# IseanB/SensorFusion-KalmanFilter

Measured on AMD Instinct MI355X. Metric: KF predict+update steps/sec (batched filters), higher is better.
Workload: dtype f64

## Files before the change

include/kf.h:

```cpp
#ifndef KFMI_KF_H
#define KFMI_KF_H

#include <stdint.h>

#ifdef __cplusplus
extern "C" {
#endif

#define KF_OK        0
#define KF_EINVAL   (-1)
#define KF_EHIP     (-2)
#define KF_ENOTSPD  (-3)
#define KF_ENODEV   (-4)
#define KF_ENOMEM   (-5)

#define KF_F32 0
#define KF_F64 1

#define KF_MODEL_CV2 2
#define KF_MODEL_CV3 3

#define KF_MODEL_REF15 15

#define KF_MODEL_REF8 8
// ... 104 lines not shown
#define KF_SCORE_IMU_N        3
#define KF_SCORE_IMU_NIS      4
#define KF_SCORE_IMU_LOGDET_S 5
#define KF_SCORE_POS_N        6
#define KF_SCORE_POS_SSE      7
#define KF_SCORE_ROWS         8
int kf_run_sweep_scores(kf_batch* handle, int T, const uint8_t* etype, const double* dt, const void* payload,
                        const double* thresholds, const double* consts, const double* track, double* scores,
                        void* traj, void* logdet, uint8_t* updated, int32_t* n_updated,
                        int ckpt_every, void* ckpt_x, void* ckpt_P, void* stream);

int kf_smooth_sweep(kf_batch* handle, int T, const uint8_t* etype, const double* dt, const double* consts,
                    const void* filt_x, const void* filt_P, void* sm_x, void* sm_P, void* sm_traj,
                    void* sm_logdet, int32_t* sm_status, void* stream);

int kf_consts_rows(int model, int* rows);

int kf_run_tails(kf_batch* handle, int T, const uint8_t* etype, const double* dt, const void* payload,
                 const int32_t* lo, const int32_t* hi, const double* thresholds,
                 const void* src_x, const void* src_P, int src_rows, int64_t src_batch,
                 const int32_t* src_row, const int32_t* src_col,
                 int32_t* n_updated, void* stream);

int kf_stream_check(kf_batch* handle, double* out, void* stream);

int kf_eval_combos(kf_batch* handle, int n_events, const double* events, const double* init,
                   double prev_time, double target_end, int k, uint64_t combo_offset, void* logdets,
                   void* max_logdet, int32_t* n_records, void* stream);

int kf_search_combos(kf_batch* handle, int n_events, const double* events, const double* init,
// ... 82 lines not shown
```

sensorfusion-kalmanfilter_amd/csrc/kf_capi.cpp:

```cpp
#include <hip/hip_runtime.h>

#include <algorithm>
#include <cmath>
#include <climits>
#include <cstdarg>
#include <cstdlib>
#include <cstdio>
#include <cstring>
#include <mutex>
#include <string>
#include <vector>

#include "../../include/kf.h"
#include "kf_internal.h"

struct kf_batch {
    int model;
    int axes;
    int n, m, c;
    int np;
    int dtype;
    int64_t B;
    int device;
    kf_params params;
// ... 34 lines not shown
    int64_t search_info[4];
    uint64_t* search_host;
    uint64_t* search_host_dev;
    bool search_ctr_zero;
    hipStream_t search_ctr_stream;
    void* win_ws;
    size_t win_ws_bytes;
    bool win_ws_graph;
    uint64_t* win_host;
    uint64_t* win_host_dev;
    size_t win_host_words;
    void* tails_ws;
    size_t tails_ws_bytes;
    bool tails_ws_graph;
    std::vector<kfmi::TailSpec> tails_host;
    void* sch_ws;
    size_t sch_ws_bytes;
    bool sch_ws_graph;
    uint64_t* sch_host;
    uint64_t* sch_host_dev;
    std::vector<double> sch_cand;
};

namespace {

thread_local std::string g_err;

int fail(int code, const char* fmt, ...) __attribute__((format(printf, 2, 3)));
int fail(int code, const char* fmt, ...) {
    char buf[512];
// ... 293 lines not shown
        case KF_OPT_STREAM_CHUNKS: ok = value == 0 || (value >= 2 && value <= (int64_t(1) << 24)); break;
        case KF_OPT_START_THREADS: ok = value == 0 || (value >= 1 && value <= kfmi::kBlock); break;
        case KF_OPT_SEARCH_KERNEL: ok = value >= 0 && value <= 2; break;
        default: return fail(KF_EINVAL, "kf_set_option: unknown option %d", option);
    }
    if (!ok) return fail(KF_EINVAL, "kf_set_option: value %lld out of range for option %d", (long long)value, option);
    h->opt[option] = value;
    return KF_OK;
}

int kf_get_option(const kf_batch* h, int option, int64_t* value) {
    if (int rc = check_handle(h)) return rc;
    if (option < 1 || option >= KF_OPT_COUNT) return fail(KF_EINVAL, "kf_get_option: unknown option %d", option);
    if (!value) return fail(KF_EINVAL, "kf_get_option: null output");
    *value = h->opt[option];
    return KF_OK;
}

const char* kf_last_error(void) { return g_err.c_str(); }

int kf_default_params(int model, kf_params* out) {
    const int d = model_axes(model);
    if (!d) return fail(KF_EINVAL, "unknown model %d", model);
    if (!out) return fail(KF_EINVAL, "null params");
    std::memset(out, 0, sizeof *out);
    if (is_ref(model)) {
        ref_default_consts(model, out);
        return KF_OK;
    }
    out->q_pos = 5.0;
// ... 143 lines not shown
    if (h->P) (void)hipFree(h->P);
    if (h->status) (void)hipFree(h->status);
    if (h->ws) (void)hipFree(h->ws);
    if (h->ws_evt) (void)hipEventDestroy(h->ws_evt);
    if (h->search_ws) (void)hipFree(h->search_ws);
    if (h->search_host) (void)hipHostFree(h->search_host);
    if (h->win_ws) (void)hipFree(h->win_ws);
    if (h->win_host) (void)hipHostFree(h->win_host);
    if (h->flag) (void)hipFree(h->flag);
    if (h->stream_ws) (void)hipFree(h->stream_ws);
    if (h->pend_u) (void)hipFree(h->pend_u);
    if (h->pend_done) (void)hipEventDestroy(h->pend_done);
    if (h->kc) (void)hipFree(h->kc);
    if (h->sched_ws) (void)hipFree(h->sched_ws);
    if (h->tails_ws) (void)hipFree(h->tails_ws);
    if (h->sch_ws) (void)hipFree(h->sch_ws);
    if (h->sch_host) (void)hipHostFree(h->sch_host);
    for (auto& r : h->retired) (void)hipFree(r.first);
    delete h;
    return KF_OK;
}

int kf_release_retired(kf_batch* h, int64_t* bytes_freed) {
    if (int rc = check_handle(h)) return rc;
    int64_t freed = 0;
    for (auto& r : h->retired) {
        (void)hipFree(r.first);
        freed += static_cast<int64_t>(r.second);
    }
    h->retired.clear();
// ... 379 lines not shown
    return run_sweep_impl("kf_run_sweep_params", h, T, etype, dt, payload, thresholds, consts, traj, logdet, updated,
                          n_updated, ckpt_every, ckpt_x, ckpt_P, stream);
}

int kf_run_sweep_scores(kf_batch* h, int T, const uint8_t* etype, const double* dt, const void* payload,
                        const double* thresholds, const double* consts, const double* track, double* scores,
                        void* traj, void* logdet, uint8_t* updated, int32_t* n_updated, int ckpt_every, void* ckpt_x,
                        void* ckpt_P, void* stream) {
    if (int rc = check_handle(h)) return rc;
    if (!consts) return fail(KF_EINVAL, "kf_run_sweep_scores: null consts (a table is mandatory; equal columns for one set)");
    if (!scores) return fail(KF_EINVAL, "kf_run_sweep_scores: null scores");
    return run_sweep_impl("kf_run_sweep_scores", h, T, etype, dt, payload, thresholds, consts, traj, logdet, updated,
                          n_updated, ckpt_every, ckpt_x, ckpt_P, stream, track, scores);
}

int kf_smooth_sweep(kf_batch* h, int T, const uint8_t* etype, const double* dt, const double* consts,
                    const void* filt_x, const void* filt_P, void* sm_x, void* sm_P, void* sm_traj, void* sm_logdet,
                    int32_t* sm_status, void* stream) {
    const char* fn = "kf_smooth_sweep";
    if (int rc = check_handle(h)) return rc;
    if (!is_ref(h)) return fail(KF_EINVAL, "%s: needs a KF_MODEL_REF15 or KF_MODEL_REF8 handle", fn);
    if (h->dtype != KF_F64) return fail(KF_EINVAL, "%s: needs an f64 handle (the f32 smoother is not built)", fn);
    if (T < 0) return fail(KF_EINVAL, "%s: T = %d < 0", fn, T);
    if (T == 0 || h->B == 0) return KF_OK;
    if (!etype || !dt || !filt_x || !filt_P) return fail(KF_EINVAL, "%s: null etype/dt/filt_x/filt_P", fn);
    if (uint64_t(T) * 8u >= (uint64_t(1) << 32))
        return fail(KF_EINVAL, "%s: T = %d events exceed the 4 GiB dt descriptor (8 T)", fn, T);
    if (uint64_t(h->B) * 27u * 8u >= (uint64_t(1) << 31))
        return fail(KF_EINVAL, "%s: B = %lld filters exceed the 2 GiB row span (27 B 8)", fn, (long long)h->B);
    const int model = h->model == KF_MODEL_REF15 ? 15 : 8;
// ... 2 lines not shown
                    kfmi::consts_rows(model));
    kfmi::SmoothArgs a{};
    a.B = h->B;
    a.T = T;
    a.etype = etype;
    a.dt = dt;
    a.filt_x = filt_x;
    a.filt_P = filt_P;
    a.sm_x = sm_x;
    a.sm_P = sm_P;
    a.sm_traj = sm_traj;
    a.sm_logdet = sm_logdet;
    a.sm_status = sm_status;
    a.kc = h->kc;
    a.consts = consts;
    hipError_t e = kfmi::launch_ref_smooth(model, a, static_cast<hipStream_t>(stream));
    return e == hipSuccess ? KF_OK : hip_fail(e, fn);
}

int kf_consts_rows(int model, int* rows) {
    if (!is_ref(model))
        return fail(KF_EINVAL, "kf_consts_rows: model %d has no per-filter constants (KF_MODEL_REF15 or KF_MODEL_REF8)",
                    model);
    if (!rows) return fail(KF_EINVAL, "kf_consts_rows: null rows");
    *rows = kfmi::consts_rows(model == KF_MODEL_REF15 ? 15 : 8);
    return KF_OK;
}

int kf_run_tails(kf_batch* h, int T, const uint8_t* etype, const double* dt, const void* payload, const int32_t* lo,
                 const int32_t* hi, const double* thresholds, const void* src_x, const void* src_P, int src_rows,
                 int64_t src_batch, const int32_t* src_row, const int32_t* src_col, int32_t* n_updated, void* stream) {
    if (int rc = check_handle(h)) return rc;
// ... 1106 lines not shown
```

sensorfusion-kalmanfilter_amd/csrc/kf_internal.h:

```cpp
#pragma once

#include <hip/hip_runtime.h>
#include <stdint.h>

namespace kfmi {

struct CvArgs {
    int64_t B;
    int T;
    int update_every;
    double dt;
    const double* dt_steps;
    const double* dt_filter;
    void* x;
    void* P;
    int32_t* status;
    const void* u;
    const void* x0;
    const void* z;
    const uint8_t* mask;
    void* traj;
    void* logdet;
    double q_pos, q_vel;
    double r[6];
// ... 95 lines not shown
};
static_assert(sizeof(int64_t) == sizeof(double*), "scores shares src_B's slot");
enum : int {
    kScoreGpsN = 0,
    kScoreGpsNis = 1,
    kScoreGpsLogdetS = 2,
    kScoreImuN = 3,
    kScoreImuNis = 4,
    kScoreImuLogdetS = 5,
    kScorePosN = 6,
    kScorePosSse = 7,
    kScoreRows = 8
};
constexpr int consts_rows(int model) { return model == 15 ? 33 : 18; }

struct SmoothArgs {
    int64_t B;
    int T;
    const uint8_t* etype;
    const double* dt;
    const void* filt_x;
    const void* filt_P;
    void* sm_x;
    void* sm_P;
    void* sm_traj;
    void* sm_logdet;
    int32_t* sm_status;
    const RefConsts* kc;
    const double* consts;
};

struct StreamCheck {
    int32_t ok;
    int32_t bad;
    double cov_gap;
    double state_gap;
    int32_t done;
    int32_t pad;
    int32_t skip_chain;
    int32_t skip_gated;
};
struct StreamArgs {
    int64_t C;
    double delta;
// ... 208 lines not shown
    bool rec_time;
};

enum class Op { Run, Predict, Update, Step, Reset };

hipError_t launch_cv(int axes, bool f64, Op op, const CvArgs& a, hipStream_t stream);
hipError_t launch_cv_offblock(int axes, bool f64, const CvArgs& a, int* flag, hipStream_t stream);
hipError_t launch_synth(int axes, bool f64, const SynthArgs& a, hipStream_t stream);
hipError_t launch_copy(void* dst, const void* src, size_t bytes, hipStream_t stream);
constexpr int kEventsLane = 0, kEventsChain = 1, kEventsLds = 2, kEventsGated = 3;
hipError_t launch_ref_events(int model, bool f64, const RefArgs& a, hipStream_t stream, int variant);
hipError_t launch_ref_stream(int model, bool f64, const RefArgs& a, hipStream_t stream, int nv = 1);
hipError_t launch_ref_sweep(int model, bool f64, const SweepArgs& a, hipStream_t stream, bool scored = false);
hipError_t launch_ref_tails(int model, bool f64, const SweepArgs& a, hipStream_t stream);
hipError_t launch_ref_smooth(int model, const SmoothArgs& a, hipStream_t stream);
hipError_t launch_ref_reset(int model, bool f64, const RefArgs& a, hipStream_t stream);
hipError_t launch_ref15_combos(bool f64, const Ref15ComboArgs& a, hipStream_t stream);
hipError_t launch_ref15_search(bool f64, const Ref15SearchArgs& a, bool child_major, hipStream_t stream);
hipError_t launch_ref15_search_pair(bool f64, const Ref15SearchArgs& a, bool child_major, hipStream_t stream);
void set_search_band(Ref15SearchArgs& a, bool f64);
hipError_t launch_ref15_search_head(bool f64, const Ref15SearchArgs& a, hipStream_t stream);
hipError_t launch_ref15_search_end(bool f64, const Ref15SearchArgs& a, hipStream_t stream);
hipError_t launch_ref15_search_windows(bool f64, bool sym, const Ref15WindowArgs* wins, int W, uint64_t max_lanes,
                                       int n_max, int k_max, const uint64_t* binom, const RefConsts* kc,
                                       hipStream_t stream);
hipError_t launch_search_windows_finish(const Ref15WindowArgs* wins, int W, int k_max, uint64_t* host,
                                        hipStream_t stream);
hipError_t launch_search_finish(uint64_t* counters, uint64_t* host, int n, bool zero, hipStream_t stream);
hipError_t launch_ref15_score(bool f64, const Ref15ScoreArgs& a, hipStream_t stream);
hipError_t launch_ref15_scheduled(bool f64, const Ref15SchedArgs& a, hipStream_t stream);
// ... 10 lines not shown
```

sensorfusion-kalmanfilter_amd/csrc/kf_ref.hip:

```cpp
#include <hip/hip_runtime.h>
#include <stdint.h>

#include <cmath>
#include <cstdlib>
#include <cstring>
#include <type_traits>

#include "kf_common.h"
#include "kf_internal.h"

namespace kfmi {
namespace {

template <typename T>
__device__ __forceinline__ __attribute__((address_space(4))) const T* ro(const T* p) {
    return (__attribute__((address_space(4))) const T*)p;
}
typedef __attribute__((address_space(4))) const double ro_double;
typedef __attribute__((address_space(4))) const uint64_t ro_u64;

using namespace dev;

constexpr int kGps = 0, kImu = 1;
constexpr int kRefNewton = 1;
// ... 1256 lines not shown
        row[kScorePosSse] = group_sum(pva ? sc.sse : 0.0);
        const auto rs = span_rsrc(a.scores, 0, uint32_t(a.B) * 8u, kScoreRows);
#pragma unroll
        for (int r = 0; r < kScoreRows; ++r) {
            const bool count = r == kScoreGpsN || r == kScoreImuN || r == kScorePosN;
            stv(rs, c == 0 ? (uint32_t(r) * uint32_t(a.B) + uint32_t(f)) * 8u : kDropOffset,
                bad && !count ? nan : row[r]);
        }
    }
}

#ifndef KF_SMOOTH_DEPTH
#define KF_SMOOTH_DEPTH KF_SWEEP_DEPTH
#endif
constexpr int kSmoothDepth = KF_SMOOTH_DEPTH;

template <typename T>
struct SmoothIn {
    int type;
    double dt;
    T x[3], P[6];
};

template <bool PARAMS>
__device__ __forceinline__ auto smooth_consts(const SmoothArgs& a, int64_t f) {
    if constexpr (PARAMS) return ConstsColumn{a.consts, a.B, f};
    else return a.kc;
}

template <typename T, class M, bool CUSTOM, bool PARAMS = false>
__global__ __launch_bounds__(kSweepBlock) void ref_smooth_kernel(const SmoothArgs a) {
    static_assert(!PARAMS || !CUSTOM, "per-filter constants in place of the handle's");
    const int64_t g = static_cast<int64_t>(blockIdx.x) * kSweepBlock + threadIdx.x;
    const int64_t f = g / kGroup;
    if (f >= a.B) return;
    const ChainLane<T, M, CUSTOM> L(static_cast<int>(g % kGroup), smooth_consts<PARAMS>(a, f));
    const int c = L.c;
    const bool live = L.live;
    const uint32_t off = uint32_t(f) * uint32_t(sizeof(T));
    const uint32_t rb = uint32_t(a.B) * uint32_t(sizeof(T));
    uint32_t vx[3], vp[6];
#pragma unroll
    for (int k = 0; k < 3; ++k) vx[k] = L.xi[k] >= 0 ? uint32_t(L.xi[k]) * rb + off : kDropOffset;
#pragma unroll
    for (int k = 0; k < 6; ++k) vp[k] = L.pr[k] >= 0 ? uint32_t(L.pr[k]) * rb + off : kDropOffset;
    const uint32_t v_tr = (L.xi[0] >= 0 && L.xi[0] < M::NTRAJ) ? uint32_t(L.xi[0]) * rb + off : kDropOffset;
    const uint32_t v_ld = c == 0 ? off : kDropOffset;
    const bool need_x = a.sm_x != nullptr, need_P = a.sm_P != nullptr;
    const bool need_tr = a.sm_traj != nullptr, need_ld = a.sm_logdet != nullptr;

    const int T_ = a.T;
    const uint32_t S = uint32_t(T_);
    const auto r_et = bytes_rsrc(a.etype, S), r_dt = bytes_rsrc(a.dt, S * 8u);
    auto load_row = [&](int t, T (&x)[3], T (&P)[6]) {
        const auto rx = span_rsrc(a.filt_x, int64_t(t) * M::N, rb, M::N);
        const auto rp = span_rsrc(a.filt_P, int64_t(t) * M::NBLK, rb, M::NBLK);
#pragma unroll
        for (int k = 0; k < 3; ++k) x[k] = ldv(rx, vx[k], T(0));
#pragma unroll
        for (int k = 0; k < 6; ++k) P[k] = L.pr[k] >= 0 ? ldv(rp, vp[k], T(0)) : L.unit(k);
    };
    auto is_nan_row = [&](const T (&x)[3], const T (&P)[6]) {
        bool nan = false;
#pragma unroll
        for (int k = 0; k < 3; ++k) nan = nan || x[k] != x[k];
#pragma unroll
        for (int k = 0; k < 6; ++k) nan = nan || P[k] != P[k];
        return nan;
    };
    int32_t st = 0;
    T xs[1][3], Ps[6];
    auto poison = [&]() {
        st = kNotSpd;
#pragma unroll
        for (int k = 0; k < 3; ++k) xs[0][k] = quiet_nan<T>();
#pragma unroll
        for (int k = 0; k < 6; ++k) Ps[k] = quiet_nan<T>();
    };
    auto store_row = [&](int t) {
        if (need_x) {
            const auto rx = span_rsrc(a.sm_x, int64_t(t) * M::N, rb, M::N);
#pragma unroll
            for (int k = 0; k < 3; ++k) stv(rx, vx[k], xs[0][k]);
        }
        if (need_P) {
            const auto rp = span_rsrc(a.sm_P, int64_t(t) * M::NBLK, rb, M::NBLK);
#pragma unroll
            for (int k = 0; k < 6; ++k) stv(rp, vp[k], Ps[k]);
        }
        if (need_tr) stv(span_rsrc(a.sm_traj, int64_t(t) * M::NTRAJ, rb, M::NTRAJ), v_tr, xs[0][0]);
        if (need_ld) {
            const T ld = group_sum(live ? chain_log_det(Ps) : T(0));
            stv(span_rsrc(a.sm_logdet, t, rb, 1), v_ld, ld);
        }
    };

    load_row(T_ - 1, xs[0], Ps);
    __builtin_amdgcn_s_waitcnt(0);
    if (group_any(live && is_nan_row(xs[0], Ps))) poison();
    store_row(T_ - 1);

    const int n = T_ - 1;
    auto load = [&](int s, SmoothIn<T>& in) {
        const int t = T_ - 2 - (s < n ? s : n - 1);
        in.type = int(__builtin_amdgcn_raw_buffer_load_b8(r_et, uint32_t(t + 1), 0, 0));
        in.dt = ldv(r_dt, uint32_t(t + 1) * 8u, 0.0);
        load_row(t, in.x, in.P);
    };
    auto step = [&](int s, const SmoothIn<T>& in) {
        const int t = T_ - 2 - s;
        const int type = wave_uniform(in.type);
        bool bad = is_nan_row(in.x, in.P);
        if (type != 255) {
            const T dt = T(in.dt);
            T xp[1][3] = {{in.x[0], in.x[1], in.x[2]}};
            T Pp[6], FP[3][3];
#pragma unroll
            for (int k = 0; k < 6; ++k) Pp[k] = in.P[k];
            L.template predict<1>(dt, xp, Pp, FP);
            const T d0 = Pp[0];
            const T i0 = T(1) / d0;
            const T l10 = Pp[1] * i0, l20 = Pp[2] * i0;
            const T v0 = l10 * d0;
            const T d1 = fmaT(-l10, v0, Pp[3]);
            const T i1 = T(1) / d1;
            const T l21 = fmaT(-l20, v0, Pp[4]) * i1;
            const T d2 = fmaT(-l21, l21 * d1, fmaT(-l20, l20 * d0, Pp[5]));
            const T i2 = T(1) / d2;
            bad = bad || !(d0 > T(0) && d1 > T(0) && d2 > T(0));
            T C[3][3];
#pragma unroll
            for (int i = 0; i < 3; ++i) {
                const T w0 = FP[0][i];
                const T w1 = fmaT(-l10, w0, FP[1][i]);
                const T w2 = fmaT(-l21, w1, fmaT(-l20, w0, FP[2][i]));
                const T c2 = w2 * i2;
                const T c1 = fmaT(-l21, c2, w1 * i1);
                const T c0 = fmaT(-l20, c2, fmaT(-l10, c1, w0 * i0));
                C[i][0] = c0, C[i][1] = c1, C[i][2] = c2;
            }
            T dx[3], D[6];
#pragma unroll
            for (int k = 0; k < 3; ++k) dx[k] = xs[0][k] - xp[0][k];
#pragma unroll
            for (int k = 0; k < 6; ++k) D[k] = Ps[k] - Pp[k];
#pragma unroll
            for (int i = 0; i < 3; ++i)
                xs[0][i] = fmaT(C[i][2], dx[2], fmaT(C[i][1], dx[1], fmaT(C[i][0], dx[0], in.x[i])));
            T CD[3][3];
#pragma unroll
            for (int i = 0; i < 3; ++i)
#pragma unroll
                for (int j = 0; j < 3; ++j)
                    CD[i][j] = fmaT(C[i][2], D[tri<3>(2, j)], fmaT(C[i][1], D[tri<3>(1, j)], C[i][0] * D[tri<3>(0, j)]));
#pragma unroll
            for (int i = 0; i < 3; ++i)
#pragma unroll
                for (int j = i; j < 3; ++j)
                    Ps[tri<3>(i, j)] =
                        fmaT(CD[i][2], C[j][2], fmaT(CD[i][1], C[j][1], fmaT(CD[i][0], C[j][0], in.P[tri<3>(i, j)])));
            if (!L.pva) {
                xs[0][2] = T(0);
                Ps[2] = Ps[4] = T(0);
                Ps[5] = T(1);
            }
        }
        if (group_any(live && bad) || st != 0) poison();
        store_row(t);
    };
    ring_run<kSmoothDepth, T, SmoothIn<T>>(n, load, step);
    if (a.sm_status) {
        const auto rs = span_rsrc(a.sm_status, 0, uint32_t(a.B) * 4u, 1);
        __builtin_amdgcn_raw_buffer_store_b32(uint32_t(st), rs, c == 0 ? uint32_t(f) * 4u : kDropOffset, 0, 0);
    }
}

template <typename T, class M, bool CUSTOM>
__global__ __launch_bounds__(64) void ref_chain_gated_kernel(const RefArgs a) {
    if (a.skip && *a.skip) return;
    const int lane = int(threadIdx.x);
    const int slot = lane / kGroup;
    const ChainLane<T, M, CUSTOM> L(lane & (kGroup - 1), a.kc);
    const int c = L.c, ia = L.ia, ib = L.ib;
    const bool pva = L.pva, live = L.live;
    const auto& xi = L.xi;
    const auto& pr = L.pr;
// ... 2969 lines not shown
    if (scored && (!a.consts || !a.scores)) return hipErrorInvalidValue;
    const dim3 grid(static_cast<unsigned>((a.B * kGroup + kSweepBlock - 1) / kSweepBlock));
    if (a.consts && scored)
        KF_MODEL_DISPATCH(model, f64,
                          ref_sweep_kernel<T, M, false, false, true, true><<<grid, kSweepBlock, 0, stream>>>(a));
    else if (a.consts)
        KF_MODEL_DISPATCH(model, f64, ref_sweep_kernel<T, M, false, false, true><<<grid, kSweepBlock, 0, stream>>>(a));
    else
        KF_REF_DISPATCH(model, f64, a.kc, ref_sweep_kernel<T, M, CUSTOM><<<grid, kSweepBlock, 0, stream>>>(a));
    return hipGetLastError();
}

hipError_t launch_ref_smooth(int model, const SmoothArgs& a, hipStream_t stream) {
    if (a.B <= 0 || a.T <= 0 || (model != 15 && model != 8) || !a.filt_x || !a.filt_P || !a.etype || !a.dt)
        return hipErrorInvalidValue;
    const dim3 grid(static_cast<unsigned>((a.B * kGroup + kSweepBlock - 1) / kSweepBlock));
    if (a.consts)
        KF_MODEL_DISPATCH(model, true, if constexpr (sizeof(T) == 8)
                                           ref_smooth_kernel<T, M, false, true><<<grid, kSweepBlock, 0, stream>>>(a));
    else
        KF_REF_DISPATCH(model, true, a.kc, if constexpr (sizeof(T) == 8)
                                               ref_smooth_kernel<T, M, CUSTOM><<<grid, kSweepBlock, 0, stream>>>(a));
    return hipGetLastError();
}

template <typename T, class M>
void stream_phase(int phase, const StreamArgs& a, hipStream_t stream) {
    constexpr int NCH = M::NP + M::NA;
    auto grid = [](int64_t n) { return dim3(static_cast<unsigned>((n + kBlock - 1) / kBlock)); };
    switch (phase) {
        case 0: stream_init_kernel<T, M><<<grid(a.C), kBlock, 0, stream>>>(a); break;
        case 1: stream_perturb_kernel<T, M><<<grid(4 * a.C), kBlock, 0, stream>>>(a); break;
        case kStreamPhaseScanTiles: {
            const dim3 g(unsigned((a.C + kScanTile - 1) / kScanTile), NCH);
            stream_scan_tiles_kernel<T, M><<<g, kScanTile, 0, stream>>>(a);
            break;
        }
// ... 303 lines not shown
```

sensorfusion-kalmanfilter_amd/kfmi/_lib.py:

```python
from __future__ import annotations

import ctypes
import glob
import hashlib
import os
import re

HERE = os.path.dirname(os.path.abspath(__file__))
LIB_PATH = os.path.abspath(os.environ.get('KFMI_LIB') or os.path.join(HERE, 'libkfmi.so'))
HEADER = os.path.normpath(os.path.join(HERE, '..', '..', 'include', 'kf.h'))
CSRC = os.path.normpath(os.path.join(HERE, '..', 'csrc'))

KF_OK = 0
KF_EINVAL = -1
KF_EHIP = -2
KF_ENOTSPD = -3
KF_ENODEV = -4
KF_ENOMEM = -5
KF_F32 = 0
KF_F64 = 1
KF_MODEL_CV2 = 2
KF_MODEL_CV3 = 3
KF_MODEL_REF15 = 15
KF_MODEL_REF8 = 8
# ... 82 lines not shown
    'kf_set_state': (_i, [_vp, _vp, _vp, _i, _vp]),
    'kf_get_state': (_i, [_vp, _vp, _vp, _i, _vp]),
    'kf_get_status': (_i, [_vp, _vp, _i, _vp]),
    'kf_predict': (_i, [_vp, _d, _vp, _vp, _vp, _vp]),
    'kf_update': (_i, [_vp, _vp, _vp, _vp, _vp]),
    'kf_run': (_i, [_vp, _i, _d, _vp, _vp, _vp, _vp, _i, _vp, _vp, _vp]),
    'kf_synth': (_i, [_vp, ctypes.c_uint64, _i64, _i, _d, _i, _vp, _vp, _vp, _vp]),
    'kf_run_events': (_i, [_vp, _i, _vp, _vp, _vp, _vp, _vp, _vp, _vp, _i, _d, _vp]),
    'kf_run_events_seq': (_i, [_vp, _i, _vp, _vp, _vp, _vp, _vp, _vp, _vp, _i, _d, _vp]),
    'kf_run_events_gates': (_i, [_vp, _i, _vp, _vp, _vp, _vp, _vp, _vp, _vp, _vp, _vp]),
    'kf_run_stream': (_i, [_vp, _i, _vp, _vp, _vp, _vp, _vp, _vp, _vp, _i, _i, _vp]),
    'kf_run_sweep': (_i, [_vp, _i, _vp, _vp, _vp, _vp, _vp, _vp, _vp, _vp, _i, _vp, _vp, _vp]),
    'kf_run_sweep_params': (_i, [_vp, _i, _vp, _vp, _vp, _vp, _vp, _vp, _vp, _vp, _vp, _i, _vp, _vp, _vp]),
    'kf_run_sweep_scores': (_i, [_vp, _i, _vp, _vp, _vp, _vp, _vp, _vp, _vp, _vp, _vp, _vp, _vp, _i, _vp, _vp, _vp]),
    'kf_smooth_sweep': (_i, [_vp, _i, _vp, _vp, _vp, _vp, _vp, _vp, _vp, _vp, _vp, _vp, _vp]),
    'kf_consts_rows': (_i, [_i, ctypes.POINTER(_i)]),
    'kf_run_tails': (_i, [_vp, _i, _vp, _vp, _vp, _vp, _vp, _vp, _vp, _vp, _i, _i64, _vp, _vp, _vp, _vp]),
    'kf_stream_check': (_i, [_vp, _vp, _vp]),
    'kf_eval_combos': (_i, [_vp, _i, _vp, _vp, _d, _d, _i, ctypes.c_uint64, _vp, _vp, _vp, _vp]),
    'kf_search_combos': (_i, [_vp, _i, _vp, _vp, _d, _d, _d, _i, _i, _i, ctypes.c_uint64,
                              ctypes.POINTER(ctypes.c_uint64), ctypes.POINTER(_i), _vp, _vp, _vp]),
    'kf_search_windows': (_i, [_vp, _i, _i, _vp, _vp, _vp, _vp, _vp, _vp, _i, _vp, _vp, _vp, _vp]),
    'kf_search_schedules': (_i, [_vp, _i, _vp, _vp, _vp, _vp, _d, _i, _vp, ctypes.POINTER(ctypes.c_uint64),
                                 ctypes.POINTER(_d), ctypes.POINTER(ctypes.c_uint64), _vp, _vp]),
    'kf_schedule_plan': (_i, [_vp, _i, _vp, _i, _vp]),
    'kf_search_plan': (_i,[_vp, _i, _vp, _i, ctypes.c_uint64, _i, _vp]),
    'kf_search_info': (_i, [_vp, _vp]),
    'kf_score_candidates': (_i, [_vp, _i, _vp, _i, _vp, _vp, _vp]),
    'kf_score_rows': (_i, [_vp, _i, _vp, _vp, _vp, _vp, _vp]),
    'kf_run_scheduled': (_i, [_vp, _i, _vp, _vp, _vp, _vp, _vp, _d, _vp, _vp, _vp, _vp, _vp]),
# ... 89 lines not shown
```

sensorfusion-kalmanfilter_amd/kfmi/engine.py:

```python
from __future__ import annotations

import collections
import ctypes
import math

import numpy as np
import torch

from . import _lib
from ._lib import KFError, check

MODELS = {
    'cv2': (_lib.KF_MODEL_CV2, 4, 2, 2, 10),
    'cv3': (_lib.KF_MODEL_CV3, 6, 3, 3, 21),
    'ref15': (_lib.KF_MODEL_REF15, 15, 3, 0, 27),
    'ref8': (_lib.KF_MODEL_REF8, 8, 2, 0, 15),
}
REF_MODELS = ('ref15', 'ref8')
TRAJ_WIDTH = {'ref15': 6, 'ref8': 3}
DTYPES = {'f32': (_lib.KF_F32, torch.float32, np.float32), 'f64': (_lib.KF_F64, torch.float64, np.float64)}


OPTIONS = {
    'predict': (_lib.KF_OPT_PREDICT, {'auto': 0, 'deferred': 0, 'eager': 1}),
# ... 122 lines not shown
            raise KFError(_lib.KF_EINVAL, 'BatchedKF is closed')
        return self._h

    def _stream(self):
        return ctypes.c_void_p(torch.cuda.current_stream(self.device).cuda_stream)

    def set_option(self, name, value):
        opt, names = OPTIONS[name]
        v = names[value] if isinstance(value, str) else int(value)
        check(_lib.lib().kf_set_option(self.handle, opt, v))
        return self

    def get_option(self, name):
        out = ctypes.c_int64(0)
        check(_lib.lib().kf_get_option(self.handle, OPTIONS[name][0], ctypes.byref(out)))
        return out.value

    def empty(self, *shape, dtype=None):
        return torch.empty(shape, dtype=dtype or self.torch_dtype, device=self.device)

    def _dev(self, a, shape, name, dtype=None):
        dt = dtype or self.torch_dtype
        if isinstance(a, np.ndarray):
            a = torch.from_numpy(np.ascontiguousarray(a))
        if not torch.is_tensor(a):
            raise TypeError(f'{name}: expected a torch tensor or numpy array, got {type(a)}')
        if tuple(a.shape) != tuple(shape):
            raise ValueError(f'{name}: shape {tuple(a.shape)} != expected {tuple(shape)}')
        if a.dtype != dt:
            raise TypeError(f'{name}: dtype {a.dtype} != expected {dt}')
# ... 602 lines not shown
```

Baseline: 55.60 billion.

## Precompute RTS smoother gains in parallel over time tiles before the sequential backward pass

Splits the reference-model RTS smoother into two kernels. A gain kernel computes the predicted state, covariance and smoother gain for every time step of a tile in parallel across steps and filters, writing them to a workspace. The backward kernel then only applies the cheap recursive update, carrying the state between tiles through a small buffer. This removes the per-step predict and Cholesky work from the serial critical path, at the cost of extra global-memory traffic, a workspace of up to about 256 MiB and more kernel launches.

```diff
diff --git a/include/kf.h b/include/kf.h
--- a/include/kf.h
+++ b/include/kf.h
@@ -142,6 +142,9 @@
                     const void* filt_x, const void* filt_P, void* sm_x, void* sm_P, void* sm_traj,
                     void* sm_logdet, int32_t* sm_status, void* stream);
 
+int kf_smooth_set_tile(kf_batch* handle, int64_t events);
+int kf_smooth_get_tile(const kf_batch* handle, int64_t* events);
+
 int kf_consts_rows(int model, int* rows);
 
 int kf_run_tails(kf_batch* handle, int T, const uint8_t* etype, const double* dt, const void* payload,
diff --git a/sensorfusion-kalmanfilter_amd/csrc/kf_capi.cpp b/sensorfusion-kalmanfilter_amd/csrc/kf_capi.cpp
--- a/sensorfusion-kalmanfilter_amd/csrc/kf_capi.cpp
+++ b/sensorfusion-kalmanfilter_amd/csrc/kf_capi.cpp
@@ -72,6 +72,10 @@
     size_t tails_ws_bytes;
     bool tails_ws_graph;
     std::vector<kfmi::TailSpec> tails_host;
+    void* smooth_ws;
+    size_t smooth_ws_bytes;
+    bool smooth_ws_graph;
+    int64_t smooth_tile;
     void* sch_ws;
     size_t sch_ws_bytes;
     bool sch_ws_graph;
@@ -395,6 +399,21 @@
     if (option < 1 || option >= KF_OPT_COUNT) return fail(KF_EINVAL, "kf_get_option: unknown option %d", option);
     if (!value) return fail(KF_EINVAL, "kf_get_option: null output");
     *value = h->opt[option];
+    return KF_OK;
+}
+
+int kf_smooth_set_tile(kf_batch* h, int64_t events) {
+    if (int rc = check_handle(h)) return rc;
+    if (events < 0 || events > INT32_MAX)
+        return fail(KF_EINVAL, "kf_smooth_set_tile: %lld events out of range (0 .. 2^31 - 1)", (long long)events);
+    h->smooth_tile = events;
+    return KF_OK;
+}
+
+int kf_smooth_get_tile(const kf_batch* h, int64_t* events) {
+    if (int rc = check_handle(h)) return rc;
+    if (!events) return fail(KF_EINVAL, "kf_smooth_get_tile: null output");
+    *events = h->smooth_tile;
     return KF_OK;
 }
 
@@ -568,6 +587,7 @@
     if (h->kc) (void)hipFree(h->kc);
     if (h->sched_ws) (void)hipFree(h->sched_ws);
     if (h->tails_ws) (void)hipFree(h->tails_ws);
+    if (h->smooth_ws) (void)hipFree(h->smooth_ws);
     if (h->sch_ws) (void)hipFree(h->sch_ws);
     if (h->sch_host) (void)hipHostFree(h->sch_host);
     for (auto& r : h->retired) (void)hipFree(r.first);
@@ -977,6 +997,8 @@
                           n_updated, ckpt_every, ckpt_x, ckpt_P, stream, track, scores);
 }
 
+static constexpr uint64_t kSmoothWsCap = uint64_t(1) << 28;
+
 int kf_smooth_sweep(kf_batch* h, int T, const uint8_t* etype, const double* dt, const double* consts,
                     const void* filt_x, const void* filt_P, void* sm_x, void* sm_P, void* sm_traj, void* sm_logdet,
                     int32_t* sm_status, void* stream) {
@@ -1009,8 +1031,35 @@
     a.sm_status = sm_status;
     a.kc = h->kc;
     a.consts = consts;
-    hipError_t e = kfmi::launch_ref_smooth(model, a, static_cast<hipStream_t>(stream));
-    return e == hipSuccess ? KF_OK : hip_fail(e, fn);
+    const int64_t steps = int64_t(T) - 1;
+    const uint64_t row = uint64_t(h->B) * kfmi::kSmoothLanes * 16u;
+    const uint64_t per_event = row * kfmi::kSmoothGainRows;
+    if (per_event >= (uint64_t(1) << 32))
+        return fail(KF_EINVAL, "%s: B = %lld filters exceed the 4 GiB gain row span (14 * 128 B)", fn, (long long)h->B);
+    int64_t tile = h->smooth_tile;
+    if (tile == 0) tile = std::max<int64_t>(1, int64_t(kSmoothWsCap / per_event));
+    tile = std::max<int64_t>(1, std::min(tile, steps));
+    const hipStream_t st = static_cast<hipStream_t>(stream);
+    const size_t need = size_t(row) * kfmi::kSmoothCarryRows + size_t(per_event) * size_t(tile);
+    if (!grow_ws(h, &h->smooth_ws, &h->smooth_ws_bytes, &h->smooth_ws_graph, need, st))
+        return capturing(st) ? fail(KF_EINVAL, "%s: the workspace (%zu bytes) must be sized by an eager call before a "
+                                               "graph capture", fn, need)
+                             : fail(KF_EHIP, "%s: cannot allocate %zu bytes of workspace (tiles of %lld events)",
+                                    fn, need, (long long)tile);
+    if (capturing(st)) h->smooth_ws_graph = true;
+    a.carry = static_cast<double*>(h->smooth_ws);
+    a.gain = a.carry + size_t(row / 8u) * kfmi::kSmoothCarryRows;
+    int64_t hi = steps;
+    do {
+        const int64_t lo = std::max<int64_t>(0, hi - tile);
+        a.t_lo = int(lo);
+        a.t_hi = int(hi);
+        hipError_t e = lo < hi ? kfmi::launch_ref_smooth_gain(model, a, st) : hipSuccess;
+        if (e == hipSuccess) e = kfmi::launch_ref_smooth(model, a, st);
+        if (e != hipSuccess) return hip_fail(e, fn);
+        hi = lo;
+    } while (hi > 0);
+    return KF_OK;
 }
 
 int kf_consts_rows(int model, int* rows) {
diff --git a/sensorfusion-kalmanfilter_amd/csrc/kf_internal.h b/sensorfusion-kalmanfilter_amd/csrc/kf_internal.h
--- a/sensorfusion-kalmanfilter_amd/csrc/kf_internal.h
+++ b/sensorfusion-kalmanfilter_amd/csrc/kf_internal.h
@@ -133,6 +133,9 @@
 };
 constexpr int consts_rows(int model) { return model == 15 ? 33 : 18; }
 
+constexpr int kSmoothLanes = 8;
+constexpr int kSmoothGainRows = 14;
+constexpr int kSmoothCarryRows = 5;
 struct SmoothArgs {
     int64_t B;
     int T;
@@ -147,6 +150,9 @@
     int32_t* sm_status;
     const RefConsts* kc;
     const double* consts;
+    int t_lo, t_hi;
+    double* gain;
+    double* carry;
 };
 
 struct StreamCheck {
@@ -385,6 +391,7 @@
 hipError_t launch_ref_sweep(int model, bool f64, const SweepArgs& a, hipStream_t stream, bool scored = false);
 hipError_t launch_ref_tails(int model, bool f64, const SweepArgs& a, hipStream_t stream);
 hipError_t launch_ref_smooth(int model, const SmoothArgs& a, hipStream_t stream);
+hipError_t launch_ref_smooth_gain(int model, const SmoothArgs& a, hipStream_t stream);
 hipError_t launch_ref_reset(int model, bool f64, const RefArgs& a, hipStream_t stream);
 hipError_t launch_ref15_combos(bool f64, const Ref15ComboArgs& a, hipStream_t stream);
 hipError_t launch_ref15_search(bool f64, const Ref15SearchArgs& a, bool child_major, hipStream_t stream);
diff --git a/sensorfusion-kalmanfilter_amd/csrc/kf_ref.hip b/sensorfusion-kalmanfilter_amd/csrc/kf_ref.hip
--- a/sensorfusion-kalmanfilter_amd/csrc/kf_ref.hip
+++ b/sensorfusion-kalmanfilter_amd/csrc/kf_ref.hip
@@ -1294,13 +1294,15 @@
 #define KF_SMOOTH_DEPTH KF_SWEEP_DEPTH
 #endif
 constexpr int kSmoothDepth = KF_SMOOTH_DEPTH;
+constexpr int kSmoothGainBlock = 256;
+static_assert(kSmoothLanes == kGroup, "the workspace rows hold one pair of doubles per lane of a group");
 
 template <typename T>
 struct SmoothIn {
-    int type;
-    double dt;
-    T x[3], P[6];
+    static constexpr int kC = 0, kXp = 9, kPp = 11, kX = 17, kP = 20, kFlag = 26, kPairs = 14;
+    T g[2 * kPairs];
 };
+static_assert(SmoothIn<double>::kPairs == kSmoothGainRows, "one workspace row per pair");
 
 template <bool PARAMS>
 __device__ __forceinline__ auto smooth_consts(const SmoothArgs& a, int64_t f) {
@@ -1308,13 +1310,136 @@
     else return a.kc;
 }
 
+template <typename T>
+__device__ __forceinline__ bool smooth_nan_row(const T (&x)[3], const T (&P)[6]) {
+    bool nan = false;
+#pragma unroll
+    for (int k = 0; k < 3; ++k) nan = nan || x[k] != x[k];
+#pragma unroll
+    for (int k = 0; k < 6; ++k) nan = nan || P[k] != P[k];
+    return nan;
+}
+
+template <typename T, class Lane>
+__device__ __forceinline__ bool smooth_gain(const Lane& L, T dt, const T (&x)[3], const T (&P)[6], T (&xp)[1][3],
+                                            T (&Pp)[6], T (&C)[3][3]) {
+    bool bad = smooth_nan_row(x, P);
+    T FP[3][3];
+#pragma unroll
+    for (int k = 0; k < 3; ++k) xp[0][k] = x[k];
+#pragma unroll
+    for (int k = 0; k < 6; ++k) Pp[k] = P[k];
+    L.template predict<1>(dt, xp, Pp, FP);
+    const T d0 = Pp[0];
+    const T i0 = T(1) / d0;
+    const T l10 = Pp[1] * i0, l20 = Pp[2] * i0;
+    const T v0 = l10 * d0;
+    const T d1 = fmaT(-l10, v0, Pp[3]);
+    const T i1 = T(1) / d1;
+    const T l21 = fmaT(-l20, v0, Pp[4]) * i1;
+    const T d2 = fmaT(-l21, l21 * d1, fmaT(-l20, l20 * d0, Pp[5]));
+    const T i2 = T(1) / d2;
+    bad = bad || !(d0 > T(0) && d1 > T(0) && d2 > T(0));
+#pragma unroll
+    for (int i = 0; i < 3; ++i) {
+        const T w0 = FP[0][i];
+        const T w1 = fmaT(-l10, w0, FP[1][i]);
+        const T w2 = fmaT(-l21, w1, fmaT(-l20, w0, FP[2][i]));
+        const T c2 = w2 * i2;
+        const T c1 = fmaT(-l21, c2, w1 * i1);
+        const T c0 = fmaT(-l20, c2, fmaT(-l10, c1, w0 * i0));
+        C[i][0] = c0, C[i][1] = c1, C[i][2] = c2;
+    }
+    return bad;
+}
+
+template <typename T, class M, class Lane>
+__device__ __forceinline__ void smooth_load_row(const Lane& L, const void* rec_x, const void* rec_P, int t, uint32_t rb,
+                                                const uint32_t (&vx)[3], const uint32_t (&vp)[6], T (&x)[3],
+                                                T (&P)[6]) {
+    const auto rx = span_rsrc(rec_x, int64_t(t) * M::N, rb, M::N);
+    const auto rp = span_rsrc(rec_P, int64_t(t) * M::NBLK, rb, M::NBLK);
+#pragma unroll
+    for (int k = 0; k < 3; ++k) x[k] = ldv(rx, vx[k], T(0));
+#pragma unroll
+    for (int k = 0; k < 6; ++k) P[k] = L.pr[k] >= 0 ? ldv(rp, vp[k], T(0)) : L.unit(k);
+}
+
+typedef unsigned int v4u __attribute__((ext_vector_type(4)));
+typedef double v2d __attribute__((ext_vector_type(2)));
+__device__ __forceinline__ void smooth_ws_ld(__amdgpu_buffer_rsrc_t r, uint32_t lane16, uint32_t rb16, int k, double& v0,
+                                             double& v1) {
+    const v2d v = __builtin_bit_cast(v2d, (v4u)__builtin_amdgcn_raw_buffer_load_b128(r, lane16, uint32_t(k) * rb16, 0));
+    v0 = v.x, v1 = v.y;
+}
+__device__ __forceinline__ void smooth_ws_st(__amdgpu_buffer_rsrc_t r, uint32_t lane16, uint32_t rb16, int k, double v0,
+                                             double v1) {
+    v2d v;
+    v.x = v0, v.y = v1;
+    __builtin_amdgcn_raw_buffer_store_b128(__builtin_bit_cast(v4u, v), r, lane16, uint32_t(k) * rb16, 0);
+}
+
 template <typename T, class M, bool CUSTOM, bool PARAMS = false>
+__global__ __launch_bounds__(kSmoothGainBlock) void ref_smooth_gain_kernel(const SmoothArgs a) {
+    static_assert(!PARAMS || !CUSTOM, "per-filter constants in place of the handle's");
+    static_assert(sizeof(T) == 8, "the workspace rows are doubles");
+    constexpr int kWaves = kSmoothGainBlock / 64;
+    const int64_t nw = (a.B * kGroup + 63) / 64;
+    const int64_t w = static_cast<int64_t>(blockIdx.x) * kWaves + wave_uniform(int(threadIdx.x) / 64);
+    const int64_t tl = w / nw;
+    if (tl >= a.t_hi - a.t_lo) return;
+    const int64_t g = (w % nw) * 64 + (threadIdx.x & 63);
+    const int64_t f = g / kGroup;
+    if (f >= a.B) return;
+    const int t = a.t_lo + int(tl);
+    const uint32_t S = uint32_t(a.T);
+    const int type = wave_uniform(int(__builtin_amdgcn_raw_buffer_load_b8(bytes_rsrc(a.etype, S), uint32_t(t + 1), 0, 0)));
+    const ChainLane<T, M, CUSTOM> L(static_cast<int>(g % kGroup), smooth_consts<PARAMS>(a, f));
+    const uint32_t off = uint32_t(f) * uint32_t(sizeof(T));
+    const uint32_t rb = uint32_t(a.B) * uint32_t(sizeof(T));
+    uint32_t vx[3], vp[6];
+#pragma unroll
+    for (int k = 0; k < 3; ++k) vx[k] = L.xi[k] >= 0 ? uint32_t(L.xi[k]) * rb + off : kDropOffset;
+#pragma unroll
+    for (int k = 0; k < 6; ++k) vp[k] = L.pr[k] >= 0 ? uint32_t(L.pr[k]) * rb + off : kDropOffset;
+    const T dt = T(ldv(bytes_rsrc(a.dt, S * 8u), uint32_t(t + 1) * 8u, 0.0));
+    T x[3], P[6];
+    smooth_load_row<T, M>(L, a.filt_x, a.filt_P, t, rb, vx, vp, x, P);
+    using In = SmoothIn<T>;
+    const uint32_t rb16 = uint32_t(a.B) * uint32_t(kGroup * 16), lane16 = uint32_t(g) * 16u;
+    const auto rg = span_rsrc(a.gain, tl * kSmoothGainRows, rb16, kSmoothGainRows);
+    if (type == 255) {
+        smooth_ws_st(rg, lane16, rb16, In::kFlag / 2, group_any(L.live && smooth_nan_row(x, P)) ? 3.0 : 2.0, 0.0);
+        return;
+    }
+    T xp[1][3], Pp[6], C[3][3];
+    const bool bad = smooth_gain(L, dt, x, P, xp, Pp, C);
+    T v[2 * In::kPairs];
+#pragma unroll
+    for (int i = 0; i < 3; ++i)
+#pragma unroll
+        for (int j = 0; j < 3; ++j) v[In::kC + 3 * i + j] = C[i][j];
+#pragma unroll
+    for (int k = 0; k < 2; ++k) v[In::kXp + k] = xp[0][k];
+#pragma unroll
+    for (int k = 0; k < 6; ++k) v[In::kPp + k] = Pp[k];
+#pragma unroll
+    for (int k = 0; k < 3; ++k) v[In::kX + k] = x[k];
+#pragma unroll
+    for (int k = 0; k < 6; ++k) v[In::kP + k] = P[k];
+    v[In::kFlag] = group_any(L.live && bad) ? 1.0 : 0.0;
+    v[In::kFlag + 1] = 0.0;
+#pragma unroll
+    for (int k = 0; k < In::kPairs; ++k) smooth_ws_st(rg, lane16, rb16, k, v[2 * k], v[2 * k + 1]);
+}
+
+template <typename T, class M>
 __global__ __launch_bounds__(kSweepBlock) void ref_smooth_kernel(const SmoothArgs a) {
-    static_assert(!PARAMS || !CUSTOM, "per-filter constants in place of the handle's");
+    static_assert(sizeof(T) == 8, "the workspace rows are doubles");
     const int64_t g = static_cast<int64_t>(blockIdx.x) * kSweepBlock + threadIdx.x;
     const int64_t f = g / kGroup;
     if (f >= a.B) return;
-    const ChainLane<T, M, CUSTOM> L(static_cast<int>(g % kGroup), smooth_consts<PARAMS>(a, f));
+    const ChainLane<T, M, false> L(static_cast<int>(g % kGroup), static_cast<const RefConsts*>(nullptr));
     const int c = L.c;
     const bool live = L.live;
     const uint32_t off = uint32_t(f) * uint32_t(sizeof(T));
@@ -1330,24 +1455,11 @@
     const bool need_tr = a.sm_traj != nullptr, need_ld = a.sm_logdet != nullptr;
 
     const int T_ = a.T;
-    const uint32_t S = uint32_t(T_);
-    const auto r_et = bytes_rsrc(a.etype, S), r_dt = bytes_rsrc(a.dt, S * 8u);
     auto load_row = [&](int t, T (&x)[3], T (&P)[6]) {
-        const auto rx = span_rsrc(a.filt_x, int64_t(t) * M::N, rb, M::N);
-        const auto rp = span_rsrc(a.filt_P, int64_t(t) * M::NBLK, rb, M::NBLK);
-#pragma unroll
-        for (int k = 0; k < 3; ++k) x[k] = ldv(rx, vx[k], T(0));
-#pragma unroll
-        for (int k = 0; k < 6; ++k) P[k] = L.pr[k] >= 0 ? ldv(rp, vp[k], T(0)) : L.unit(k);
+        smooth_load_row<T, M>(L, a.filt_x, a.filt_P, t, rb, vx, vp, x, P);
     };
-    auto is_nan_row = [&](const T (&x)[3], const T (&P)[6]) {
-        bool nan = false;
-#pragma unroll
-        for (int k = 0; k < 3; ++k) nan = nan || x[k] != x[k];
-#pragma unroll
-        for (int k = 0; k < 6; ++k) nan = nan || P[k] != P[k];
-        return nan;
-    };
+    const uint32_t rb16 = uint32_t(a.B) * uint32_t(kGroup * 16), lane16 = uint32_t(g) * 16u;
+    const auto r_carry = span_rsrc(a.carry, 0, rb16, kSmoothCarryRows);
     int32_t st = 0;
     T xs[1][3], Ps[6];
     auto poison = [&]() {
@@ -1375,58 +1487,50 @@
         }
     };
 
-    load_row(T_ - 1, xs[0], Ps);
-    __builtin_amdgcn_s_waitcnt(0);
-    if (group_any(live && is_nan_row(xs[0], Ps))) poison();
-    store_row(T_ - 1);
-
-    const int n = T_ - 1;
-    auto load = [&](int s, SmoothIn<T>& in) {
-        const int t = T_ - 2 - (s < n ? s : n - 1);
-        in.type = int(__builtin_amdgcn_raw_buffer_load_b8(r_et, uint32_t(t + 1), 0, 0));
-        in.dt = ldv(r_dt, uint32_t(t + 1) * 8u, 0.0);
-        load_row(t, in.x, in.P);
+    const int t_lo = a.t_lo, t_hi = a.t_hi;
+    if (t_hi == T_ - 1) {
+        load_row(T_ - 1, xs[0], Ps);
+        __builtin_amdgcn_s_waitcnt(0);
+        if (group_any(live && smooth_nan_row(xs[0], Ps))) poison();
+        store_row(T_ - 1);
+    } else {
+        T v[2 * kSmoothCarryRows];
+#pragma unroll
+        for (int k = 0; k < kSmoothCarryRows; ++k) smooth_ws_ld(r_carry, lane16, rb16, k, v[2 * k], v[2 * k + 1]);
+#pragma unroll
+        for (int k = 0; k < 3; ++k) xs[0][k] = v[k];
+#pragma unroll
+        for (int k = 0; k < 6; ++k) Ps[k] = v[3 + k];
+        st = int32_t(v[9]);
+    }
+
+    const int n = t_hi - t_lo;
+    using In = SmoothIn<T>;
+    auto load = [&](int s, In& in) {
+        const int t = t_hi - 1 - (s < n ? s : n - 1);
+        const auto rg = span_rsrc(a.gain, int64_t(t - t_lo) * kSmoothGainRows, rb16, kSmoothGainRows);
+#pragma unroll
+        for (int k = 0; k < In::kPairs; ++k) smooth_ws_ld(rg, lane16, rb16, k, in.g[2 * k], in.g[2 * k + 1]);
     };
-    auto step = [&](int s, const SmoothIn<T>& in) {
-        const int t = T_ - 2 - s;
-        const int type = wave_uniform(in.type);
-        bool bad = is_nan_row(in.x, in.P);
-        if (type != 255) {
-            const T dt = T(in.dt);
-            T xp[1][3] = {{in.x[0], in.x[1], in.x[2]}};
-            T Pp[6], FP[3][3];
-#pragma unroll
-            for (int k = 0; k < 6; ++k) Pp[k] = in.P[k];
-            L.template predict<1>(dt, xp, Pp, FP);
-            const T d0 = Pp[0];
-            const T i0 = T(1) / d0;
-            const T l10 = Pp[1] * i0, l20 = Pp[2] * i0;
-            const T v0 = l10 * d0;
-            const T d1 = fmaT(-l10, v0, Pp[3]);
-            const T i1 = T(1) / d1;
-            const T l21 = fmaT(-l20, v0, Pp[4]) * i1;
-            const T d2 = fmaT(-l21, l21 * d1, fmaT(-l20, l20 * d0, Pp[5]));
-            const T i2 = T(1) / d2;
-            bad = bad || !(d0 > T(0) && d1 > T(0) && d2 > T(0));
-            T C[3][3];
-#pragma unroll
-            for (int i = 0; i < 3; ++i) {
-                const T w0 = FP[0][i];
-                const T w1 = fmaT(-l10, w0, FP[1][i]);
-                const T w2 = fmaT(-l21, w1, fmaT(-l20, w0, FP[2][i]));
-                const T c2 = w2 * i2;
-                const T c1 = fmaT(-l21, c2, w1 * i1);
-                const T c0 = fmaT(-l20, c2, fmaT(-l10, c1, w0 * i0));
-                C[i][0] = c0, C[i][1] = c1, C[i][2] = c2;
-            }
-            T dx[3], D[6];
-#pragma unroll
-            for (int k = 0; k < 3; ++k) dx[k] = xs[0][k] - xp[0][k];
-#pragma unroll
-            for (int k = 0; k < 6; ++k) D[k] = Ps[k] - Pp[k];
+    auto step = [&](int s, const In& in) {
+        const int t = t_hi - 1 - s;
+        const int flag = int(in.g[In::kFlag]);
+        const bool gbad = (flag & 1) != 0;
+        if (wave_uniform(flag >> 1) == 0) {
+            T C[3][3], dx[3], D[6];
 #pragma unroll
             for (int i = 0; i < 3; ++i)
-                xs[0][i] = fmaT(C[i][2], dx[2], fmaT(C[i][1], dx[1], fmaT(C[i][0], dx[0], in.x[i])));
+#pragma unroll
+                for (int j = 0; j < 3; ++j) C[i][j] = in.g[In::kC + 3 * i + j];
+            const T* x_f = &in.g[In::kX];
+            const T* P_f = &in.g[In::kP];
+#pragma unroll
+            for (int k = 0; k < 3; ++k) dx[k] = xs[0][k] - (k < 2 ? in.g[In::kXp + k] : x_f[2]);
+#pragma unroll
+            for (int k = 0; k < 6; ++k) D[k] = Ps[k] - in.g[In::kPp + k];
+#pragma unroll
+            for (int i = 0; i < 3; ++i)
+                xs[0][i] = fmaT(C[i][2], dx[2], fmaT(C[i][1], dx[1], fmaT(C[i][0], dx[0], x_f[i])));
             T CD[3][3];
 #pragma unroll
             for (int i = 0; i < 3; ++i)
@@ -1438,18 +1542,24 @@
 #pragma unroll
                 for (int j = i; j < 3; ++j)
                     Ps[tri<3>(i, j)] =
-                        fmaT(CD[i][2], C[j][2], fmaT(CD[i][1], C[j][1], fmaT(CD[i][0], C[j][0], in.P[tri<3>(i, j)])));
+                        fmaT(CD[i][2], C[j][2], fmaT(CD[i][1], C[j][1], fmaT(CD[i][0], C[j][0], P_f[tri<3>(i, j)])));
             if (!L.pva) {
                 xs[0][2] = T(0);
                 Ps[2] = Ps[4] = T(0);
                 Ps[5] = T(1);
             }
         }
-        if (group_any(live && bad) || st != 0) poison();
+        if (gbad || st != 0) poison();
         store_row(t);
     };
     ring_run<kSmoothDepth, T, SmoothIn<T>>(n, load, step);
-    if (a.sm_status) {
+    if (t_lo > 0) {
+        smooth_ws_st(r_carry, lane16, rb16, 0, xs[0][0], xs[0][1]);
+        smooth_ws_st(r_carry, lane16, rb16, 1, xs[0][2], Ps[0]);
+        smooth_ws_st(r_carry, lane16, rb16, 2, Ps[1], Ps[2]);
+        smooth_ws_st(r_carry, lane16, rb16, 3, Ps[3], Ps[4]);
+        smooth_ws_st(r_carry, lane16, rb16, 4, Ps[5], double(st));
+    } else if (a.sm_status) {
         const auto rs = span_rsrc(a.sm_status, 0, uint32_t(a.B) * 4u, 1);
         __builtin_amdgcn_raw_buffer_store_b32(uint32_t(st), rs, c == 0 ? uint32_t(f) * 4u : kDropOffset, 0, 0);
     }
@@ -4449,13 +4559,28 @@
 hipError_t launch_ref_smooth(int model, const SmoothArgs& a, hipStream_t stream) {
     if (a.B <= 0 || a.T <= 0 || (model != 15 && model != 8) || !a.filt_x || !a.filt_P || !a.etype || !a.dt)
         return hipErrorInvalidValue;
+    if (a.t_lo < 0 || a.t_lo > a.t_hi || a.t_hi > a.T - 1 || !a.gain || !a.carry) return hipErrorInvalidValue;
     const dim3 grid(static_cast<unsigned>((a.B * kGroup + kSweepBlock - 1) / kSweepBlock));
+    KF_MODEL_DISPATCH(model, true, if constexpr (sizeof(T) == 8)
+                                       ref_smooth_kernel<T, M><<<grid, kSweepBlock, 0, stream>>>(a));
+    return hipGetLastError();
+}
+
+hipError_t launch_ref_smooth_gain(int model, const SmoothArgs& a, hipStream_t stream) {
+    if (a.B <= 0 || a.T <= 0 || (model != 15 && model != 8) || !a.filt_x || !a.filt_P || !a.etype || !a.dt)
+        return hipErrorInvalidValue;
+    if (a.t_lo < 0 || a.t_lo >= a.t_hi || a.t_hi > a.T - 1 || !a.gain) return hipErrorInvalidValue;
+    constexpr int64_t kWaves = kSmoothGainBlock / 64;
+    const int64_t waves = int64_t(a.t_hi - a.t_lo) * ((a.B * kGroup + 63) / 64);
+    const int64_t blocks = (waves + kWaves - 1) / kWaves;
+    if (blocks > INT32_MAX) return hipErrorInvalidValue;
+    const dim3 grid(static_cast<unsigned>(blocks));
     if (a.consts)
-        KF_MODEL_DISPATCH(model, true, if constexpr (sizeof(T) == 8)
-                                           ref_smooth_kernel<T, M, false, true><<<grid, kSweepBlock, 0, stream>>>(a));
+        KF_MODEL_DISPATCH(model, true, if constexpr (sizeof(T) == 8) ref_smooth_gain_kernel<T, M, false, true>
+                                       <<<grid, kSmoothGainBlock, 0, stream>>>(a));
     else
-        KF_REF_DISPATCH(model, true, a.kc, if constexpr (sizeof(T) == 8)
-                                               ref_smooth_kernel<T, M, CUSTOM><<<grid, kSweepBlock, 0, stream>>>(a));
+        KF_REF_DISPATCH(model, true, a.kc, if constexpr (sizeof(T) == 8) ref_smooth_gain_kernel<T, M, CUSTOM>
+                                           <<<grid, kSmoothGainBlock, 0, stream>>>(a));
     return hipGetLastError();
 }
 
diff --git a/sensorfusion-kalmanfilter_amd/kfmi/_lib.py b/sensorfusion-kalmanfilter_amd/kfmi/_lib.py
--- a/sensorfusion-kalmanfilter_amd/kfmi/_lib.py
+++ b/sensorfusion-kalmanfilter_amd/kfmi/_lib.py
@@ -120,6 +120,8 @@
     'kf_run_sweep_params': (_i, [_vp, _i, _vp, _vp, _vp, _vp, _vp, _vp, _vp, _vp, _vp, _i, _vp, _vp, _vp]),
     'kf_run_sweep_scores': (_i, [_vp, _i, _vp, _vp, _vp, _vp, _vp, _vp, _vp, _vp, _vp, _vp, _vp, _i, _vp, _vp, _vp]),
     'kf_smooth_sweep': (_i, [_vp, _i, _vp, _vp, _vp, _vp, _vp, _vp, _vp, _vp, _vp, _vp, _vp]),
+    'kf_smooth_set_tile': (_i, [_vp, _i64]),
+    'kf_smooth_get_tile': (_i, [_vp, ctypes.POINTER(_i64)]),
     'kf_consts_rows': (_i, [_i, ctypes.POINTER(_i)]),
     'kf_run_tails': (_i, [_vp, _i, _vp, _vp, _vp, _vp, _vp, _vp, _vp, _vp, _i, _i64, _vp, _vp, _vp, _vp]),
     'kf_stream_check': (_i, [_vp, _vp, _vp]),
diff --git a/sensorfusion-kalmanfilter_amd/kfmi/engine.py b/sensorfusion-kalmanfilter_amd/kfmi/engine.py
--- a/sensorfusion-kalmanfilter_amd/kfmi/engine.py
+++ b/sensorfusion-kalmanfilter_amd/kfmi/engine.py
@@ -160,6 +160,15 @@
     def get_option(self, name):
         out = ctypes.c_int64(0)
         check(_lib.lib().kf_get_option(self.handle, OPTIONS[name][0], ctypes.byref(out)))
+        return out.value
+
+    def set_smooth_tile(self, events):
+        check(_lib.lib().kf_smooth_set_tile(self.handle, int(events)))
+        return self
+
+    def get_smooth_tile(self):
+        out = ctypes.c_int64(0)
+        check(_lib.lib().kf_smooth_get_tile(self.handle, ctypes.byref(out)))
         return out.value
 
     def empty(self, *shape, dtype=None):
```

Result: slower. 48.69 billion (-12.4%).
